# InternetMaximalism/intmax-zkp-core

Measured on NVIDIA B200. Metric: LDE+Merkle commit cells/s, higher is better.
Workload: dtype u64 (Goldilocks field, 32-bit IMAD/IADD3 limbs)

## Files before the change

intmax_zkp_core_b200/csrc/b200zkp.cu:

```cuda
#include "../../include/b200zkp.h"
#include "../../include/b200zkp_test.h"

#include <cuda_runtime.h>

#include <algorithm>
#include <cstdio>
#include <cstdlib>
#include <cstring>
#include <map>
#include <memory>
#include <mutex>
#include <optional>
#include <string>
#include <tuple>
#include <vector>

#include "merkle_kernels.cuh"
#include "ntt_kernels.cuh"
#include "eval_kernels.cuh"
#include "fri_kernels.cuh"
#include "perm_kernels.cuh"
#include "vanishing_kernels.cuh"
#include "host_plan.hpp"

using gl::u32;
using gl::u64;

static inline u64 gl_host_canon(u64 a) { return a >= hostgl::P ? a - hostgl::P : a; }

struct TwoLevel {
    u64* lo = nullptr;
    u64* hi = nullptr;
    u32 lo_bits = 0;
};

struct b200zkp_ctx {
    int device = 0;
    cudaStream_t stream = nullptr;
    bool own_stream = false;
    std::mutex mu;
    std::string err;
    u64 launches = 0;
    u64* wtab[2][ntt::MAX_PASS_BITS + 1] = {};
    std::map<u32, TwoLevel> tw[2];
    struct Images { const u64* img[ntt::MAX_PASSES] = {}; };
    std::map<std::tuple<u32, int, bool>, Images> twimg;
    std::map<std::pair<u32, u32>, const u64*> coset_scale;
    std::map<std::pair<u64, u32>, const u64*> power_scale;
    struct ZTables { const u64* strided = nullptr; const u64* final_ = nullptr; };
    std::map<std::pair<u32, u32>, ZTables> ztab_lde;
    std::map<u32, ZTables> ztab_inv;
    bool ntt_ct = true;
    bool ntt_tma = true;
    u32 ct_smem_set = 0;
    u32 sm_count = 0;
    u64 coop_leaf_rows = 2048;
    u64 coop_level_nodes = 2048;
    void* mailbox = nullptr;
    void* mailbox_dev = nullptr;
    u64* round_add = nullptr;
    std::multimap<size_t, void*> pool;
    size_t pool_bytes = 0;
    size_t live_bytes = 0;
    size_t pool_max_bytes = (size_t)16 << 30;
    std::vector<void*> table_allocs;
    cudaStream_t stream2 = nullptr;
    std::vector<cudaEvent_t> sync_events;
    bool timing = false;
    std::vector<cudaEvent_t> ev_free;
    struct Span { int stage; cudaEvent_t a, b; };
    std::vector<Span> spans;
};

struct StageTimer {
    b200zkp_ctx* c;
    int stage;
    cudaEvent_t a = nullptr;
    static cudaEvent_t get(b200zkp_ctx* c) {
        cudaEvent_t e = nullptr;
        if (!c->ev_free.empty()) { e = c->ev_free.back(); c->ev_free.pop_back(); }
        else if (cudaEventCreate(&e) != cudaSuccess) { (void)cudaGetLastError(); e = nullptr; }
        return e;
    }
    StageTimer(b200zkp_ctx* ctx, int st) : c(ctx), stage(st) {
        if (c->timing && (a = get(c))) cudaEventRecord(a, c->stream);
    }
    ~StageTimer() {
        if (!a) return;
        cudaEvent_t b = get(c);
        if (b) { cudaEventRecord(b, c->stream); c->spans.push_back({stage, a, b}); }
        else c->ev_free.push_back(a);
    }
};

struct Guard {
    b200zkp_ctx* c;
    explicit Guard(b200zkp_ctx* ctx) : c(ctx) { c->mu.lock(); cudaSetDevice(c->device); }
    ~Guard() { c->mu.unlock(); }
};

struct StreamScope {
    b200zkp_ctx* c;
    cudaStream_t saved;
    StreamScope(b200zkp_ctx* ctx, cudaStream_t s) : c(ctx), saved(ctx->stream) { c->stream = s; }
    ~StreamScope() { c->stream = saved; }
};

#define CUDA_TRY(ctx, expr)                                                                   \
    do {                                                                                      \
        cudaError_t e__ = (expr);                                                             \
        if (e__ != cudaSuccess) {                                                             \
            (ctx)->err = std::string(#expr) + ": " + cudaGetErrorString(e__);                 \
            (void)cudaGetLastError();                                                         \
            return e__ == cudaErrorMemoryAllocation ? B200ZKP_ERR_OOM : B200ZKP_ERR_CUDA;     \
        }                                                                                     \
    } while (0)
#define TRY(expr) do { int rc__ = (expr); if (rc__ != 0) return rc__; } while (0)
#define BAD(ctx, msg) do { (ctx)->err = (msg); return B200ZKP_ERR_BAD_ARG; } while (0)
#define LAUNCH_CHECK(ctx) do { (ctx)->launches++; CUDA_TRY(ctx, cudaGetLastError()); } while (0)

static void pool_drop(b200zkp_ctx* ctx) {
    for (auto& kv : ctx->pool) cudaFree(kv.second);
    ctx->pool.clear();
    ctx->pool_bytes = 0;
}

class DevBuf {
  public:
    DevBuf() = default;
    DevBuf(const DevBuf&) = delete;
    DevBuf& operator=(const DevBuf&) = delete;
    DevBuf(DevBuf&& o) noexcept : ctx_(o.ctx_), p_(o.p_), bytes_(o.bytes_) { o.p_ = nullptr; o.bytes_ = 0; }
    DevBuf& operator=(DevBuf&& o) noexcept {
        if (this != &o) { reset(); ctx_ = o.ctx_; p_ = o.p_; bytes_ = o.bytes_; o.p_ = nullptr; o.bytes_ = 0; }
        return *this;
    }
    ~DevBuf() { reset(); }

    u64* get() const { return (u64*)p_; }
    size_t bytes() const { return bytes_; }

    int alloc(b200zkp_ctx* ctx, size_t bytes) {
        reset();
        ctx_ = ctx;
        if (bytes == 0) return 0;
        void* p = nullptr;
        auto it = ctx->pool.find(bytes);
        if (it != ctx->pool.end()) {
            p = it->second; ctx->pool_bytes -= it->first; ctx->pool.erase(it);
        } else {
            cudaError_t e = cudaMalloc(&p, bytes);
            if (e == cudaErrorMemoryAllocation) {
                (void)cudaGetLastError();
                pool_drop(ctx);
                e = cudaMalloc(&p, bytes);
            }
            if (e != cudaSuccess) {
                ctx->err = std::string("cudaMalloc: ") + cudaGetErrorString(e);
                (void)cudaGetLastError();
                return e == cudaErrorMemoryAllocation ? B200ZKP_ERR_OOM : B200ZKP_ERR_CUDA;
            }
        }
        p_ = p; bytes_ = bytes;
        ctx->live_bytes += bytes;
        return 0;
    }
    int ensure(b200zkp_ctx* ctx, size_t bytes) { return bytes_ >= bytes ? 0 : alloc(ctx, bytes); }

    void reset() {
        if (!p_) return;
        ctx_->live_bytes -= bytes_;
        if (ctx_->pool.size() < 256 && ctx_->pool_bytes + bytes_ <= ctx_->pool_max_bytes) {
            ctx_->pool.emplace(bytes_, p_);
            ctx_->pool_bytes += bytes_;
        } else {
            cudaFree(p_);
        }
        p_ = nullptr; bytes_ = 0;
    }

  private:
    b200zkp_ctx* ctx_ = nullptr;
    void* p_ = nullptr;
    size_t bytes_ = 0;
};

struct b200zkp_batch {
    b200zkp_ctx* ctx;
    u32 n_log, k, rate_bits, cap_height, salt;
    DevBuf coeffs, lde, digests, cap;
};

struct b200zkp_tree {
    b200zkp_ctx* ctx;
    u64 n_leaves;
    u32 leaf_len, cap_height;
    DevBuf digests, cap;
};

static int d2h(b200zkp_ctx* ctx, void* dst, const void* src, size_t bytes) {
    if (!bytes) return 0;
    CUDA_TRY(ctx, cudaMemcpyAsync(dst, src, bytes, cudaMemcpyDeviceToHost, ctx->stream));
    CUDA_TRY(ctx, cudaStreamSynchronize(ctx->stream));
    return 0;
}
static int h2d(b200zkp_ctx* ctx, void* dst, const void* src, size_t bytes) {
    if (!bytes) return 0;
// ... 40 lines not shown
    auto it = cache.find(key);
    if (it == cache.end()) {
        typename Map::mapped_type t{};
        TRY(build(&t));
        it = cache.emplace(key, t).first;
    }
    *out = it->second;
    return 0;
}

static int get_tw(b200zkp_ctx* ctx, int dir, u32 n_log, TwoLevel* out) {
    return get_or_build(ctx->tw[dir], n_log, out, [&](TwoLevel* t) -> int {
        const u64 w = hostgl::root(n_log);
        std::vector<u64> lo, hi;
        t->lo_bits = hostgl::two_level_powers(dir ? hostgl::inv(w) : w, n_log, &lo, &hi);
        TRY(upload(ctx, lo, &t->lo));
        return upload(ctx, hi, &t->hi);
    });
}

static int fill_powers(b200zkp_ctx* ctx, u64 base, u32 bits, u64* dst) {
    std::vector<u64> lo, hi;
    const u32 lo_bits = hostgl::two_level_powers(base, bits, &lo, &hi);
    DevBuf d_lo, d_hi;
    TRY(d_lo.alloc(ctx, lo.size() * 8));
    TRY(d_hi.alloc(ctx, hi.size() * 8));
    TRY(h2d(ctx, d_lo.get(), lo.data(), d_lo.bytes()));
    TRY(h2d(ctx, d_hi.get(), hi.data(), d_hi.bytes()));
    const u64 n = (u64)1 << bits;
    ntt::build_powers_kernel<<<(unsigned)((n + 255) / 256), 256, 0, ctx->stream>>>(dst, n, d_lo.get(), d_hi.get(), lo_bits);
    LAUNCH_CHECK(ctx);
    CUDA_TRY(ctx, cudaStreamSynchronize(ctx->stream));
    return 0;
}

static int get_power_scale(b200zkp_ctx* ctx, u64 shift, u32 bits, const u64** out) {
    return get_or_build(ctx->power_scale, std::make_pair(shift, bits), out, [&](const u64** t) -> int {
        u64* d = nullptr;
        TRY(table_alloc(ctx, (u64)1 << bits, &d));
        *t = d;
        return fill_powers(ctx, shift, bits, d);
    });
}

static int get_coset_scale(b200zkp_ctx* ctx, u32 n_log, u32 rate_bits, const u64** out) {
    return get_or_build(ctx->coset_scale, std::make_pair(n_log, rate_bits), out, [&](const u64** t) -> int {
        const u64 n = (u64)1 << n_log;
        u64* d = nullptr;
        TRY(table_alloc(ctx, n << rate_bits, &d));
        for (u32 b = 0; b < (1u << rate_bits); b++)
            TRY(fill_powers(ctx, hostgl::coset_shift_of_block(n_log, rate_bits, b), n_log, d + (u64)b * n));
        *t = d;
        return 0;
    });
}

template <int B>
static void launch_pass_b(const ntt::PassParams& p, dim3 grid, cudaStream_t s) {
    switch (ntt::pass_mode(p)) {
        case ntt::MODE_MID_NATURAL: ntt::ntt_pass_kernel<B, ntt::MODE_MID_NATURAL><<<grid, ntt::threads_for(B), 0, s>>>(p); break;
        case ntt::MODE_MID_BITREV: ntt::ntt_pass_kernel<B, ntt::MODE_MID_BITREV><<<grid, ntt::threads_for(B), 0, s>>>(p); break;
        case ntt::MODE_FINAL_BITREV: ntt::ntt_pass_kernel<B, ntt::MODE_FINAL_BITREV><<<grid, ntt::threads_for(B), 0, s>>>(p); break;
        default: ntt::ntt_pass_kernel<B, ntt::MODE_FINAL_NATURAL><<<grid, ntt::threads_for(B), 0, s>>>(p); break;
    }
}
static int launch_pass(b200zkp_ctx* ctx, const ntt::PassParams& p, u32 B, u32 n_blk) {
    u64 T = (u64)ntt::tile_elems_for((int)B) >> B;
    u64 total_batches = (u64)p.ncols << (p.n_log - B);
    u64 blocks = (total_batches + T - 1) / T;
    if (blocks == 0 || n_blk == 0) return 0;
    if (blocks > 0x7fffffffull || n_blk > 65535) BAD(ctx, "transform too large for one launch");
    dim3 grid((unsigned)blocks, n_blk);
    switch (B) {
        case 1: launch_pass_b<1>(p, grid, ctx->stream); break;
        case 2: launch_pass_b<2>(p, grid, ctx->stream); break;
        case 3: launch_pass_b<3>(p, grid, ctx->stream); break;
        case 4: launch_pass_b<4>(p, grid, ctx->stream); break;
        case 5: launch_pass_b<5>(p, grid, ctx->stream); break;
        case 6: launch_pass_b<6>(p, grid, ctx->stream); break;
        case 7: launch_pass_b<7>(p, grid, ctx->stream); break;
        case 8: launch_pass_b<8>(p, grid, ctx->stream); break;
        case 9: launch_pass_b<9>(p, grid, ctx->stream); break;
        case 10: launch_pass_b<10>(p, grid, ctx->stream); break;
        default: BAD(ctx, "internal: bad pass width");
    }
    LAUNCH_CHECK(ctx);
    return 0;
}

static int launch_canon_copy(b200zkp_ctx* ctx, const u64* src, u64* dst, u64 count) {
    if (!count) return 0;
    ntt::canon_copy_kernel<<<(unsigned)((count + 255) / 256), 256, 0, ctx->stream>>>(src, dst, count);
    LAUNCH_CHECK(ctx);
    return 0;
}

static int get_twiddle_images(b200zkp_ctx* ctx, u32 n_log, int dir, bool bitrev_out, b200zkp_ctx::Images* out) {
    return get_or_build(ctx->twimg, std::make_tuple(n_log, dir, bitrev_out), out, [&](b200zkp_ctx::Images* im) -> int {
        ntt::TwiddleImageShape shapes[ntt::MAX_PASSES];
        u32 n_img = ntt::twiddle_images(n_log, shapes);
        if (!n_img) return 0;
        TwoLevel tw{};
        TRY(get_tw(ctx, dir, n_log, &tw));
        u64 n_inv = hostgl::inv(((u64)1 << n_log) % hostgl::P);
        for (u32 pi = 0; pi < n_img; pi++) {
            u64 count = (u64)1 << (shapes[pi].B + shapes[pi].C_log);
            u64* d = nullptr;
            TRY(table_alloc(ctx, count, &d));
            u64 f = (dir == 1 && pi == 0) ? n_inv : 0;
            ntt::build_twiddle_image_kernel<<<(unsigned)((count + 255) / 256), 256, 0, ctx->stream>>>(
                d, shapes[pi].B, shapes[pi].C_log, shapes[pi].shift, bitrev_out ? 1u : 0u, f, tw.lo, tw.hi, tw.lo_bits);
            LAUNCH_CHECK(ctx);
            im->img[pi] = d;
        }
        return 0;
    });
}

typedef CUresult (*TensorMapEncodeFn)(CUtensorMap*, CUtensorMapDataType, cuuint32_t, void*, const cuuint64_t*, const cuuint64_t*,
                                      const cuuint32_t*, const cuuint32_t*, CUtensorMapInterleave, CUtensorMapSwizzle,
                                      CUtensorMapL2promotion, CUtensorMapFloatOOBfill);
static TensorMapEncodeFn tensor_map_encoder() {
    static TensorMapEncodeFn fn = [] {
        void* p = nullptr;
        cudaDriverEntryPointQueryResult q;
        if (cudaGetDriverEntryPoint("cuTensorMapEncodeTiled", &p, cudaEnableDefault, &q) != cudaSuccess || q != cudaDriverEntryPointSuccess) {
            (void)cudaGetLastError();
            p = nullptr;
        }
        return (TensorMapEncodeFn)p;
    }();
    return fn;
}

static bool encode_tile_map(CUtensorMap* map, const u64* base, u32 B, u32 S, u32 C_log, u32 n_blk, u64 blk_stride, u32 ncols,
                            u64 col_stride) {
    TensorMapEncodeFn enc = tensor_map_encoder();
    if (!enc) return false;
    const u64 C = (u64)1 << C_log, rows = (u64)1 << B, A = (u64)1 << S;
    cuuint64_t dims[5] = {C, rows, A, n_blk ? n_blk : 1, ncols};
    cuuint64_t strides[4] = {C * 8, C * rows * 8, (blk_stride ? blk_stride : C * rows * A) * 8, col_stride * 8};
    cuuint32_t box[5] = {(cuuint32_t)(ntc::TILE >> B), (cuuint32_t)rows, 1, 1, 1};
    cuuint32_t estr[5] = {1, 1, 1, 1, 1};
    CUresult r = enc(map, CU_TENSOR_MAP_DATA_TYPE_UINT64, 5, (void*)base, dims, strides, box, estr, CU_TENSOR_MAP_INTERLEAVE_NONE,
                     CU_TENSOR_MAP_SWIZZLE_NONE, CU_TENSOR_MAP_L2_PROMOTION_L2_128B, CU_TENSOR_MAP_FLOAT_OOB_FILL_NONE);
    return r == CUDA_SUCCESS;
}

template <int B>
static int launch_ct_b(b200zkp_ctx* ctx, int kind, const ntc::PassParams& p, u64 grid, const CUtensorMap& tm_in, const CUtensorMap& tm_out,
                       const ntc::PullMaps* tm_src, const CUtensorMap* tm_copy, u32 pull_ctas_per_sm) {
    const void* fn = nullptr;
    u32 smem = 0;
    switch (kind) {
        case ntc::KIND_STRIDED: fn = (const void*)ntc::ct_pass_kernel<B, ntc::KIND_STRIDED>; smem = ntc::StridedSmem<B, false>::bytes; break;
        case ntc::KIND_STRIDED_LOOP: fn = (const void*)ntc::ct_pass_kernel<B, ntc::KIND_STRIDED_LOOP>; smem = ntc::StridedSmem<B, true>::bytes; break;
        case ntc::KIND_FINAL_INPLACE: fn = (const void*)ntc::ct_pass_kernel<B, ntc::KIND_FINAL_INPLACE>; smem = ntc::FinalSmem<B>::bytes; break;
        case ntc::KIND_PULL_LOOP: fn = (const void*)ntc::ct_pull_kernel<B>; smem = ntc::PullSmem<B>::bytes; break;
        default: fn = (const void*)ntc::ct_pass_kernel<B, ntc::KIND_FINAL_NATURAL>; smem = ntc::FinalSmem<B>::bytes; break;
    }
    const u32 bit = 1u << ((B - ntc::MIN_BITS) * 5 + kind);
    if (smem > 48 * 1024 && !(ctx->ct_smem_set & bit)) {
        CUDA_TRY(ctx, cudaFuncSetAttribute(fn, cudaFuncAttributeMaxDynamicSharedMemorySize, (int)smem));
        ctx->ct_smem_set |= bit;
    }
    void* args[5] = {(void*)&p, (void*)&tm_in, (void*)&tm_out, nullptr, nullptr};
    u32 total = (u32)grid;
    if (kind == ntc::KIND_PULL_LOOP) {
        args[1] = (void*)tm_src; args[2] = (void*)&tm_out; args[3] = (void*)tm_copy; args[4] = (void*)&total;
        if (!ctx->sm_count) {
            int sms = 0;
            CUDA_TRY(ctx, cudaDeviceGetAttribute(&sms, cudaDevAttrMultiProcessorCount, ctx->device));
            ctx->sm_count = (u32)std::max(1, sms);
        }
        grid = std::min<u64>(grid, (u64)std::max(1u, pull_ctas_per_sm) * ctx->sm_count);
    }
    CUDA_TRY(ctx, cudaLaunchKernel(fn, dim3((unsigned)grid), dim3(ntc::THREADS), args, smem, ctx->stream));
    ctx->launches++;
    return 0;
}

static int run_ct_plan(b200zkp_ctx* ctx, ntc::Plan& plan, cudaStream_t later_stream = nullptr, cudaEvent_t first_done = nullptr,
                       u32 pull_ctas_per_sm = 4) {
    cudaStream_t const first_stream = ctx->stream;
    std::optional<StreamScope> later;
    for (u32 pi = 0; pi < plan.n_passes; pi++) {
        if (pi == 1 && later_stream && later_stream != first_stream) {
            CUDA_TRY(ctx, cudaEventRecord(first_done, first_stream));
            CUDA_TRY(ctx, cudaStreamWaitEvent(later_stream, first_done, 0));
            later.emplace(ctx, later_stream);
        }
        ntc::PassParams& p = plan.pass[pi];
        const u32 B = plan.bits[pi];
        const int kind = plan.kind[pi];
        if (plan.grid[pi] > 0x7fffffffull) BAD(ctx, "transform too large for one launch");
        alignas(64) CUtensorMap tm_in, tm_out, tm_copy;
        alignas(64) ntc::PullMaps tm_src;
        memset(&tm_in, 0, sizeof tm_in); memset(&tm_out, 0, sizeof tm_out); memset(&tm_copy, 0, sizeof tm_copy);
        const bool pull = kind == ntc::KIND_PULL_LOOP;
        if (pull) memset(&tm_src, 0, sizeof tm_src);
        const u32 map_cols = p.col_run ? p.col_limit : p.ncols;
        if (p.use_tma) {
            const bool loop = kind == ntc::KIND_STRIDED_LOOP || pull;
            bool ok = ctx->ntt_tma && encode_tile_map(&tm_out, p.out, B, p.S, p.C_log, p.n_blk, p.out_blk_stride, map_cols, p.out_col_stride);
            if (ok && pull) {
                ok = encode_tile_map(&tm_copy, p.copy_out, B, p.S, p.C_log, 1, 0, map_cols, p.copy_col_stride);
                const u32 src_cols = ((p.col_limit + p.col_period - 1) / p.col_period) * p.col_run;
                for (u32 q = 0; ok && q < p.col_period / p.col_run; q++)
                    ok = encode_tile_map(&tm_src.m[q], p.src[q], B, p.S, p.C_log, 1, 0, src_cols, p.in_col_stride);
            } else if (ok) {
                ok = encode_tile_map(&tm_in, p.in, B, p.S, p.C_log, loop ? 1 : p.n_blk, loop ? 0 : p.in_blk_stride, map_cols, p.in_col_stride);
            }
            if (!ok) p.use_tma = 0;
        }
        switch (B) {
            case 5: TRY(launch_ct_b<5>(ctx, kind, p, plan.grid[pi], tm_in, tm_out, &tm_src, &tm_copy, pull_ctas_per_sm)); break;
            case 6: TRY(launch_ct_b<6>(ctx, kind, p, plan.grid[pi], tm_in, tm_out, &tm_src, &tm_copy, pull_ctas_per_sm)); break;
            case 7: TRY(launch_ct_b<7>(ctx, kind, p, plan.grid[pi], tm_in, tm_out, &tm_src, &tm_copy, pull_ctas_per_sm)); break;
            case 8: TRY(launch_ct_b<8>(ctx, kind, p, plan.grid[pi], tm_in, tm_out, &tm_src, &tm_copy, pull_ctas_per_sm)); break;
            default: BAD(ctx, "internal: bad pass width");
        }
    }
    return 0;
}

static int build_ztab(b200zkp_ctx* ctx, u32 n_log, int dir, const std::vector<u64>& shifts, u64 last_scale, bool natural,
                      b200zkp_ctx::ZTables* out) {
    TwoLevel tw{};
    TRY(get_tw(ctx, dir, n_log, &tw));
    std::vector<u64> spow((size_t)shifts.size() * n_log);
    for (size_t b = 0; b < shifts.size(); b++) {
        u64 x = shifts[b] % hostgl::P;
        for (u32 e = 0; e < n_log; e++) { spow[b * n_log + e] = x; x = hostgl::mul(x, x); }
    }
    DevBuf d_spow;
    TRY(d_spow.alloc(ctx, spow.size() * 8));
    TRY(h2d(ctx, d_spow.get(), spow.data(), d_spow.bytes()));
    const u64 count = ntc::ztab_entries(n_log), words = ntc::zfinal_words(n_log);
    u64 *d = nullptr, *f = nullptr;
    TRY(table_alloc(ctx, count * shifts.size(), &d));
    TRY(table_alloc(ctx, words * shifts.size(), &f));
    ntc::build_ztab_kernel<<<dim3((unsigned)((count + 255) / 256), (unsigned)shifts.size()), 256, 0, ctx->stream>>>(
        d, count, n_log, d_spow.get(), tw.lo, tw.hi, tw.lo_bits, last_scale);
    LAUNCH_CHECK(ctx);
    ntc::build_zfinal_kernel<<<dim3((unsigned)((words + 255) / 256), (unsigned)shifts.size()), 256, 0, ctx->stream>>>(
        f, words, n_log, ntc::last_pass_bits(n_log), natural ? 1u : 0u, d_spow.get(), tw.lo, tw.hi, tw.lo_bits, last_scale);
    LAUNCH_CHECK(ctx);
    CUDA_TRY(ctx, cudaStreamSynchronize(ctx->stream));
    out->strided = d;
    out->final_ = f;
    return 0;
}

static int get_ztab_lde(b200zkp_ctx* ctx, u32 n_log, u32 rate_bits, b200zkp_ctx::ZTables* out) {
    return get_or_build(ctx->ztab_lde, std::make_pair(n_log, rate_bits), out, [&](b200zkp_ctx::ZTables* t) {
        std::vector<u64> shifts;
        for (u32 b = 0; b < (1u << rate_bits); b++) shifts.push_back(hostgl::coset_shift_of_block(n_log, rate_bits, b));
        return build_ztab(ctx, n_log, 0, shifts, 0, false, t);
    });
}

static int get_ztab_inv(b200zkp_ctx* ctx, u32 n_log, b200zkp_ctx::ZTables* out) {
    return get_or_build(ctx->ztab_inv, n_log, out, [&](b200zkp_ctx::ZTables* t) {
        return build_ztab(ctx, n_log, 1, std::vector<u64>{1}, hostgl::inv(((u64)1 << n_log) % hostgl::P), true, t);
    });
}

static int run_transform(b200zkp_ctx* ctx, const u64* in, u64 in_stride, u64* out, u64 out_stride,
                         u64* scratch, u32 n_log, u32 ncols, int dir, bool bitrev_out,
                         const u64* scale, u64 scale_blk_stride, bool inverse_scale, bool canon_in,
                         u32 n_blk = 1, u64 out_blk_stride = 0) {
    if (ncols == 0) return 0;
    if (n_log == 0) {
        for (u32 blk = 0; blk < n_blk; blk++)
            for (u32 c = 0; c < ncols; c++)
                TRY(launch_canon_copy(ctx, in + c * in_stride, out + blk * out_blk_stride + c * out_stride, 1));
        return 0;
    }
    if (n_log > 32) BAD(ctx, "n_log exceeds the field's two-adicity (32)");
    if (!bitrev_out && n_log > (u32)ntt::MAX_PASS_BITS && !scratch) BAD(ctx, "scratch buffer required for multi-pass natural-order transforms");
    b200zkp_ctx::Images im;
    TRY(get_twiddle_images(ctx, n_log, dir, bitrev_out, &im));
    ntt::TransformTables tb{};
    tb.wtab = ctx->wtab[dir];
    for (u32 i = 0; i < ntt::MAX_PASSES; i++) tb.twimg[i] = im.img[i];
    tb.scale = scale;
    tb.scale_blk_stride = scale_blk_stride;
    u64 n_inv = hostgl::inv(((u64)1 << n_log) % hostgl::P);
    ntt::Plan plan;
    ntt::make_plan(&plan, in, in_stride, out, out_stride, scratch, n_log, ncols, tb, bitrev_out,
                   inverse_scale ? n_inv : 0, canon_in, 0, out_blk_stride);
    for (u32 pi = 0; pi < plan.n_passes; pi++) TRY(launch_pass(ctx, plan.pass[pi], plan.bits[pi], n_blk));
    return 0;
}

extern "C" const char* b200zkp_version(void) { return "b200zkp 0.1 (sm_100a)"; }

extern "C" int b200zkp_device_count(void) {
    int n = 0;
    cudaError_t e = cudaGetDeviceCount(&n);
    if (e != cudaSuccess) { (void)cudaGetLastError(); return B200ZKP_ERR_CUDA; }
    return n;
}

static int ctx_init_tables(b200zkp_ctx* ctx) {
    TRY(table_alloc(ctx, 360, &ctx->round_add));
    CUDA_TRY(ctx, cudaMemcpyFromSymbolAsync(ctx->round_add, poseidon_tables::ROUND_ADD, 360 * sizeof(u64), 0,
                                            cudaMemcpyDeviceToDevice, ctx->stream));
    for (int dir = 0; dir < 2; dir++)
        for (u32 B = 1; B <= (u32)ntt::MAX_PASS_BITS; B++) TRY(upload(ctx, hostgl::small_root_table(B, dir), &ctx->wtab[dir][B]));
    return 0;
}

extern "C" int b200zkp_ctx_create(int device, void* stream, b200zkp_ctx** out) {
// ... 1591 lines not shown
```

intmax_zkp_core_b200/csrc/ntt_ct_kernels.cuh:

```cuda
#pragma once
#include "goldilocks.cuh"

#ifndef B200ZKP_HOST_EMU
#include <cuda.h>
#endif

namespace ntc {

using gl::u32;
using gl::u64;

static constexpr int TILE = 2048;
static constexpr int THREADS = 256;
static constexpr int MIN_BITS = 5, MAX_BITS = 8;
static constexpr int MAX_LOOP_BLOCKS = 8;
static constexpr int MAX_SRC = 8;

enum Kind : int {
    KIND_STRIDED = 0,
    KIND_STRIDED_LOOP = 1,
    KIND_FINAL_INPLACE = 2,
    KIND_FINAL_NATURAL = 3,
    KIND_PULL_LOOP = 4,
};

struct PassParams {
    const u64* in;
    u64* out;
    u64 in_col_stride, out_col_stride;
    u64 in_blk_stride, out_blk_stride;
    u32 ncols, n_blk;
    u32 n_log;
    u32 S;
    u32 C_log;
    const u64* ztab;
    u64 ztab_blk_stride;
    u64 a_scale;
    u32 use_tma;
    u32 col_run, col_period, col0, col_limit, col_sel, col_src;
    const u64* src[MAX_SRC];
    u64* copy_out;
    u64 copy_col_stride;
};

GL_FN u32 map_column(const PassParams& p, u32 v, u32& q, u32& i) {
    if (p.col_run == 0) { q = 0; i = v; return v; }
    u32 phys;
    if (p.col_sel) phys = p.col0 + (v / p.col_run) * p.col_period + p.col_src * p.col_run + v % p.col_run;
    else phys = p.col0 + v;
    const u32 in_grp = phys % p.col_period;
    q = in_grp / p.col_run;
    i = (phys / p.col_period) * p.col_run + in_grp % p.col_run;
    return phys < p.col_limit ? phys : 0xFFFFFFFFu;
}

GL_FN u32 ulog2(u32 e) {
#ifdef B200ZKP_HOST_EMU
    u32 r = 0; while (e >>= 1) r++; return r;
#else
    return 31u - (u32)__clz((int)e);
#endif
}
GL_FN u32 bitrev_bits(u32 x, u32 bits) { return bits ? (gl::brev32(x) >> (32 - bits)) : 0; }

GL_FN u64 z_index(u64 prefix, u32 e) {
    const u32 u = ulog2(e);
    return (prefix << u) + (e ^ (1u << u));
}

GL_FN void butterfly(u64& a, u64& b, u64 z) {
    const u64 t = gl::canon_cc(gl::mul_nc(b, z));
    const u64 a0 = a;
    a = gl::add_nc(a0, t);
    b = gl::sub_nc(a0, t);
}

template <int A, bool SCALE>
GL_FN void ct_group(u64 (&x)[1 << A], const u64* __restrict__ tw, u32 u0, u32 gh, u64 a_scale) {
#pragma unroll
    for (int v = 0; v < A; v++) {
        const int half = (1 << A) >> (v + 1);
        u64 z[1 << (A - 1)];
#pragma unroll
        for (int q = 0; q < (1 << v); q++) z[q] = tw[(1u << (u0 + v)) + (gh << v) + q];
#pragma unroll
        for (int j = 0; j < (1 << A); j++) {
            if (j & half) continue;
            if (SCALE && v == A - 1) x[j] = gl::canon_cc(gl::mul_nc(x[j], a_scale));
            butterfly(x[j], x[j + half], z[j >> (A - v)]);
        }
    }
}

#ifdef B200ZKP_HOST_EMU
#define NTC_FOR_THREADS(tid) for (u32 tid = 0; tid < (u32)THREADS; tid++)
#define NTC_SYNC() do {} while (0)
#else
#define NTC_FOR_THREADS(tid) for (u32 tid = threadIdx.x, once__ = 1; once__; once__ = 0)
#define NTC_SYNC() __syncthreads()
#endif

template <int A, bool SCALE>
GL_FN void run_round(const u64* __restrict__ src, u64* __restrict__ dst, const u64* __restrict__ tw, u32 tw_pitch, u32 B,
                     u32 T_log, u32 pitch, u32 u0, u64 a_scale, u32 tid) {
    const u32 st_log = B - u0 - A;
    constexpr int UNITS = 8 >> A;
#pragma unroll
    for (int r = 0; r < UNITS; r++) {
        const u32 U = tid + r * THREADS;
        const u32 t = U & ((1u << T_log) - 1), w = U >> T_log;
        const u32 gl_ = w & ((1u << st_log) - 1), gh = w >> st_log;
        const u32 gbase = (gh << (st_log + A)) + gl_;
        u64 x[1 << A];
#pragma unroll
        for (int j = 0; j < (1 << A); j++) x[j] = src[(gbase + ((u32)j << st_log)) * pitch + t];
        ct_group<A, SCALE>(x, tw + t * tw_pitch, u0, gh, a_scale);
#pragma unroll
        for (int j = 0; j < (1 << A); j++) dst[(gbase + ((u32)j << st_log)) * pitch + t] = x[j];
    }
}

template <int B, bool SCALE>
GL_FN void run_rounds(const u64* first_src, u64* tile, const u64* tw, u32 tw_pitch, u32 T_log, u32 pitch, u64 a_scale) {
    u32 u0 = 0;
    const u64* src = first_src;
    if (B % 3 == 2) { NTC_FOR_THREADS(tid) { run_round<2, false>(src, tile, tw, tw_pitch, B, T_log, pitch, u0, a_scale, tid); } u0 += 2; src = tile; NTC_SYNC(); }
    if (B % 3 == 1) { NTC_FOR_THREADS(tid) { run_round<1, false>(src, tile, tw, tw_pitch, B, T_log, pitch, u0, a_scale, tid); } u0 += 1; src = tile; NTC_SYNC(); }
#pragma unroll 1
    for (int r = 0; r < B / 3 - 1; r++) {
        NTC_FOR_THREADS(tid) { run_round<3, false>(src, tile, tw, tw_pitch, B, T_log, pitch, u0, a_scale, tid); }
        u0 += 3; src = tile;
        NTC_SYNC();
    }
    NTC_FOR_THREADS(tid) { run_round<3, SCALE>(src, tile, tw, tw_pitch, B, T_log, pitch, u0, a_scale, tid); }
}

#ifndef B200ZKP_HOST_EMU
__device__ __forceinline__ u32 smem_u32(const void* p) { return (u32)__cvta_generic_to_shared(p); }
__device__ __forceinline__ void mbar_init(u64* bar, u32 count) {
    asm volatile("mbarrier.init.shared::cta.b64 [%0], %1;" ::"r"(smem_u32(bar)), "r"(count) : "memory");
}
__device__ __forceinline__ void fence_barrier_init() { asm volatile("fence.mbarrier_init.release.cluster;" ::: "memory"); }
__device__ __forceinline__ void fence_proxy_async() { asm volatile("fence.proxy.async.shared::cta;" ::: "memory"); }
__device__ __forceinline__ void mbar_expect_tx(u64* bar, u32 bytes) {
    asm volatile("mbarrier.arrive.expect_tx.shared::cta.b64 _, [%0], %1;" ::"r"(smem_u32(bar)), "r"(bytes) : "memory");
}
__device__ __forceinline__ void mbar_wait(u64* bar, u32 parity) {
    asm volatile(
        "{\n\t.reg .pred p;\n\t"
        "NTC_WAIT:\n\t"
        "mbarrier.try_wait.parity.shared::cta.b64 p, [%0], %1;\n\t"
        "@p bra NTC_DONE;\n\t"
        "bra NTC_WAIT;\n\t"
        "NTC_DONE:\n\t}" ::"r"(smem_u32(bar)), "r"(parity) : "memory");
}
__device__ __forceinline__ void tma_load_tile(void* dst, const CUtensorMap* map, u32 c0, u32 a, u32 blk, u32 col, u64* bar) {
    asm volatile("cp.async.bulk.tensor.5d.shared::cluster.global.mbarrier::complete_tx::bytes [%0], [%1, {%2, %3, %4, %5, %6}], [%7];"
                 ::"r"(smem_u32(dst)), "l"(map), "r"(c0), "r"(0u), "r"(a), "r"(blk), "r"(col), "r"(smem_u32(bar)) : "memory");
}
__device__ __forceinline__ void tma_store_tile(const CUtensorMap* map, u32 c0, u32 a, u32 blk, u32 col, const void* src) {
    asm volatile("cp.async.bulk.tensor.5d.global.shared::cta.bulk_group [%0, {%1, %2, %3, %4, %5}], [%6];"
                 ::"l"(map), "r"(c0), "r"(0u), "r"(a), "r"(blk), "r"(col), "r"(smem_u32(src)) : "memory");
}
__device__ __forceinline__ void bulk_load(void* dst, const void* src, u32 bytes, u64* bar) {
    asm volatile("cp.async.bulk.shared::cluster.global.mbarrier::complete_tx::bytes [%0], [%1], %2, [%3];"
                 ::"r"(smem_u32(dst)), "l"(src), "r"(bytes), "r"(smem_u32(bar)) : "memory");
}
__device__ __forceinline__ void tma_commit() { asm volatile("cp.async.bulk.commit_group;" ::: "memory"); }
template <int N>
__device__ __forceinline__ void tma_wait_read() { asm volatile("cp.async.bulk.wait_group.read %0;" ::"n"(N) : "memory"); }
template <int N>
__device__ __forceinline__ void tma_wait_all() { asm volatile("cp.async.bulk.wait_group %0;" ::"n"(N) : "memory"); }
#endif

template <int B, bool LOOP>
struct StridedSmem {
    static constexpr u32 NPTS = 1u << B;
    static constexpr u32 tiles = LOOP ? 3 : 1;
    static constexpr u32 sw_words = (LOOP ? (u32)MAX_LOOP_BLOCKS : 1u) * NPTS;
    static constexpr u32 bytes = tiles * TILE * 8 + sw_words * 8 + 16;
};

template <int B, bool LOOP, typename TMap, bool PULL = false>
GL_FN void strided_body(const PassParams& p, const TMap* tm_in, const TMap* tm_out, u64* smem, u32 bid, const TMap* tm_copy = nullptr) {
    static_assert(!PULL || LOOP, "a pull pass stages its tile apart from the work tiles");
    constexpr u32 NPTS = 1u << B;
    constexpr u32 T_log = 11 - B, T = 1u << T_log;
    constexpr u32 IT = TILE / THREADS;
    u64* const stage = smem;
    u64* const work0 = LOOP ? smem + TILE : smem;
    u64* const sw = smem + StridedSmem<B, LOOP>::tiles * TILE;
    u64* const bar = sw + StridedSmem<B, LOOP>::sw_words;

    const u32 V = LOOP ? p.ncols : p.ncols * p.n_blk;
    const u32 vcol = bid % V, tile_i = bid / V;
    u32 src_q, src_i;
    const u32 col = map_column(p, LOOP ? vcol : vcol / p.n_blk, src_q, src_i);
    if (col == 0xFFFFFFFFu) return;
    const u32 in_col = PULL ? src_i : col;
    const u32 blk_fixed = LOOP ? 0u : vcol % p.n_blk;
    const u32 tiles_per_a_log = p.C_log - T_log;
    const u32 a = tile_i >> tiles_per_a_log;
    const u32 c0 = (tile_i & ((1u << tiles_per_a_log) - 1)) << T_log;
    const u64 prefix = ((u64)1 << p.S) + a;
    const u64 elem0 = ((u64)a << (B + p.C_log)) + c0;
    const u64* __restrict__ in = (PULL ? p.src[src_q] : p.in) + (u64)in_col * p.in_col_stride + (u64)blk_fixed * p.in_blk_stride + elem0;
    (void)tm_in; (void)tm_out; (void)tm_copy; (void)bar;

#ifndef B200ZKP_HOST_EMU
    const bool tma = p.use_tma != 0;
    if (tma) {
        if (threadIdx.x == 0) { mbar_init(bar, 1); fence_barrier_init(); }
        __syncthreads();
        if (threadIdx.x == 0) {
            mbar_expect_tx(bar, TILE * 8);
            tma_load_tile(stage, PULL ? tm_in + src_q : tm_in, c0, a, blk_fixed, in_col, bar);
        }
    }
#else
    const bool tma = false;
#endif
    NTC_FOR_THREADS(tid) {
        const u32 nb = LOOP ? p.n_blk : 1u;
        for (u32 i = tid; i < nb * NPTS; i += THREADS) {
            const u32 b = LOOP ? i >> B : blk_fixed, e = i & (NPTS - 1);
            if (e) sw[i] = gl::ldg(p.ztab + (u64)b * p.ztab_blk_stride + z_index(prefix, e));
        }
        if (!tma) {
            u64 v[IT];
#pragma unroll
            for (u32 it = 0; it < IT; it++) {
                const u32 i = tid + it * THREADS;
                v[it] = in[((u64)(i >> T_log) << p.C_log) + (i & (T - 1))];
            }
#pragma unroll
            for (u32 it = 0; it < IT; it++) stage[tid + it * THREADS] = v[it];
            if (PULL) {
                u64* __restrict__ cp = p.copy_out + (u64)col * p.copy_col_stride + elem0;
#pragma unroll
                for (u32 it = 0; it < IT; it++) {
                    const u32 i = tid + it * THREADS;
                    cp[((u64)(i >> T_log) << p.C_log) + (i & (T - 1))] = v[it];
                }
            }
        }
    }
#ifndef B200ZKP_HOST_EMU
    if (tma) {
        mbar_wait(bar, 0);
        if (PULL && threadIdx.x == 0) { tma_store_tile(tm_copy, c0, a, 0, col, stage); tma_commit(); }
    }
#endif
    NTC_SYNC();

    const u32 n_loop = LOOP ? p.n_blk : 1u;
    for (u32 lb = 0; lb < n_loop; lb++) {
        const u32 blk = LOOP ? lb : blk_fixed;
        u64* const tile = LOOP ? work0 + (lb & 1) * TILE : work0;
#ifndef B200ZKP_HOST_EMU
        if (LOOP && tma && lb >= 2) { if (threadIdx.x == 0) tma_wait_read<1>(); __syncthreads(); }
#endif
        run_rounds<B, false>(LOOP ? stage : tile, tile, sw + (LOOP ? lb * NPTS : 0), 0, T_log, T, 0);
        u64* __restrict__ out = p.out + (u64)col * p.out_col_stride + (u64)blk * p.out_blk_stride + elem0;
#ifndef B200ZKP_HOST_EMU
        if (tma) {
            fence_proxy_async();
            __syncthreads();
            if (threadIdx.x == 0) { tma_store_tile(tm_out, c0, a, blk, col, tile); tma_commit(); }
            continue;
        }
#endif
        NTC_SYNC();
        NTC_FOR_THREADS(tid) {
#pragma unroll
            for (u32 it = 0; it < IT; it++) {
                const u32 i = tid + it * THREADS;
                out[((u64)(i >> T_log) << p.C_log) + (i & (T - 1))] = tile[i];
            }
        }
        NTC_SYNC();
    }
#ifndef B200ZKP_HOST_EMU
    if (tma && threadIdx.x == 0) tma_wait_read<0>();
#endif
}

template <int B>
struct FinalSmem {
    static constexpr u32 NPTS = 1u << B, T = (u32)TILE >> B;
    static constexpr u32 TP = T + 1, TWP = NPTS + 1;
    static constexpr u32 tw_words = T * TWP;
    static constexpr u32 bytes = (NPTS * TP + tw_words) * 8 + 16;
};

template <int B, bool NATURAL>
GL_FN void final_body(const PassParams& p, u64* smem, u32 bid) {
    constexpr u32 NPTS = 1u << B;
    constexpr u32 T_log = 11 - B, T = 1u << T_log, TP = FinalSmem<B>::TP, TWP = FinalSmem<B>::TWP;
    constexpr u32 IT = TILE / THREADS;
    u64* const tile = smem;
    u64* const swb = smem + NPTS * TP;
    u64* const bar = swb + FinalSmem<B>::tw_words;
    (void)bar;
    const u32 batches_log = p.n_log - B;
    const u32 V = p.ncols * p.n_blk;
    const u32 vcol = bid % V, tile_i = bid / V;
    u32 src_q, src_i;
    const u32 col = map_column(p, vcol / p.n_blk, src_q, src_i), blk = vcol % p.n_blk;
    if (col == 0xFFFFFFFFu) return;
    const u32 batch0 = tile_i << T_log;
    const u64* __restrict__ in = p.in + (u64)col * p.in_col_stride + (u64)blk * p.in_blk_stride;
    u64* __restrict__ out = p.out + (u64)col * p.out_col_stride + (u64)blk * p.out_blk_stride;
    const u64* __restrict__ ztile = p.ztab + (u64)blk * p.ztab_blk_stride + (u64)tile_i * FinalSmem<B>::tw_words;

#ifndef B200ZKP_HOST_EMU
    if (threadIdx.x == 0) { mbar_init(bar, 1); fence_barrier_init(); }
    __syncthreads();
    if (threadIdx.x == 0) {
        mbar_expect_tx(bar, FinalSmem<B>::tw_words * 8);
        bulk_load(swb, ztile, FinalSmem<B>::tw_words * 8, bar);
    }
#else
    for (u32 i = 0; i < FinalSmem<B>::tw_words; i++) swb[i] = ztile[i];
#endif
    NTC_FOR_THREADS(tid) {
        u64 v[IT];
#pragma unroll
        for (u32 it = 0; it < IT; it += 2) {
            const u32 i = 2 * (tid + (it / 2) * THREADS);
            const u32 b = i >> B, g = i & (NPTS - 1);
            const u32 a_b = NATURAL ? bitrev_bits(batch0 + b, batches_log) : batch0 + b;
#ifdef B200ZKP_HOST_EMU
            v[it] = in[((u64)a_b << B) + g]; v[it + 1] = in[((u64)a_b << B) + g + 1];
#else
            const ulonglong2 q = *reinterpret_cast<const ulonglong2*>(in + ((u64)a_b << B) + g);
            v[it] = q.x; v[it + 1] = q.y;
#endif
        }
#pragma unroll
        for (u32 it = 0; it < IT; it += 2) {
            const u32 i = 2 * (tid + (it / 2) * THREADS);
            const u32 b = i >> B, g = i & (NPTS - 1);
            tile[g * TP + b] = v[it];
            tile[(g + 1) * TP + b] = v[it + 1];
        }
    }
#ifndef B200ZKP_HOST_EMU
    mbar_wait(bar, 0);
#endif
    NTC_SYNC();

    if (p.a_scale) run_rounds<B, true>(tile, tile, swb, TWP, T_log, TP, p.a_scale);
    else run_rounds<B, false>(tile, tile, swb, TWP, T_log, TP, 0);
    NTC_SYNC();

    NTC_FOR_THREADS(tid) {
        if (NATURAL) {
#pragma unroll
            for (u32 it = 0; it < IT; it++) {
                const u32 i = tid + it * THREADS;
                const u32 tau = i & (T - 1), r = i >> T_log;
                const u32 g = bitrev_bits(r, B);
                out[((u64)r << batches_log) + batch0 + tau] = gl::canon_cc(tile[g * TP + tau]);
            }
        } else {
#pragma unroll
            for (u32 it = 0; it < IT; it += 2) {
                const u32 i = 2 * (tid + (it / 2) * THREADS);
                const u32 b = i >> B, g = i & (NPTS - 1);
                const u64 x0 = gl::canon_cc(tile[g * TP + b]), x1 = gl::canon_cc(tile[(g + 1) * TP + b]);
#ifdef B200ZKP_HOST_EMU
                out[((u64)(batch0 + b) << B) + g] = x0; out[((u64)(batch0 + b) << B) + g + 1] = x1;
#else
                *reinterpret_cast<ulonglong2*>(out + ((u64)(batch0 + b) << B) + g) = make_ulonglong2(x0, x1);
#endif
            }
        }
    }
}

#ifndef B200ZKP_HOST_EMU
template <int B, int KIND>
__global__ void __launch_bounds__(THREADS, 4)
ct_pass_kernel(const PassParams p, const __grid_constant__ CUtensorMap tm_in, const __grid_constant__ CUtensorMap tm_out) {
    extern __shared__ __align__(128) unsigned char ntc_smem_raw[];
    u64* smem = reinterpret_cast<u64*>(ntc_smem_raw);
    if (KIND == KIND_STRIDED) strided_body<B, false>(p, &tm_in, &tm_out, smem, blockIdx.x);
    else if (KIND == KIND_STRIDED_LOOP) strided_body<B, true>(p, &tm_in, &tm_out, smem, blockIdx.x);
    else if (KIND == KIND_FINAL_INPLACE) final_body<B, false>(p, smem, blockIdx.x);
    else final_body<B, true>(p, smem, blockIdx.x);
}

struct PullMaps { CUtensorMap m[MAX_SRC]; };
template <int B>
struct PullSmem {
    static constexpr u32 NPTS = 1u << B;
    static constexpr u32 sw_words = (u32)MAX_LOOP_BLOCKS * NPTS;
    static constexpr u32 bytes = 4 * TILE * 8 + sw_words * 8 + 32;
};

template <int B>
__device__ __forceinline__ void pull_decode(const PassParams& p, u32 bid, u32& col, u32& in_col, u32& q, u32& a, u32& c0) {
    constexpr u32 T_log = 11 - B;
    const u32 vcol = bid % p.ncols, tile_i = bid / p.ncols;
    u32 i;
    col = map_column(p, vcol, q, i);
    in_col = i;
    const u32 tiles_per_a_log = p.C_log - T_log;
    a = tile_i >> tiles_per_a_log;
    c0 = (tile_i & ((1u << tiles_per_a_log) - 1)) << T_log;
}

template <int B>
__global__ void __launch_bounds__(THREADS, 4)
ct_pull_kernel(const PassParams p, const __grid_constant__ PullMaps tm_src, const __grid_constant__ CUtensorMap tm_out,
               const __grid_constant__ CUtensorMap tm_copy, const u32 total) {
    extern __shared__ __align__(128) unsigned char ntc_smem_raw[];
    u64* const smem = reinterpret_cast<u64*>(ntc_smem_raw);
    if (!p.use_tma) {
        for (u32 bid = blockIdx.x; bid < total; bid += gridDim.x) {
            strided_body<B, true, CUtensorMap, true>(p, tm_src.m, &tm_out, smem, bid, &tm_copy);
            __syncthreads();
        }
        return;
    }
    constexpr u32 NPTS = 1u << B;
    constexpr u32 T_log = 11 - B, T = 1u << T_log;
    u64* const stage0 = smem;
    u64* const work0 = smem + 2 * TILE;
    u64* const sw = smem + 4 * TILE;
    u64* const bar = sw + PullSmem<B>::sw_words;
    if (blockIdx.x >= total) return;
    if (threadIdx.x == 0) { mbar_init(bar, 1); mbar_init(bar + 1, 1); fence_barrier_init(); }
    __syncthreads();
    u32 col, in_col, q, a, c0;
    if (threadIdx.x == 0) {
        pull_decode<B>(p, blockIdx.x, col, in_col, q, a, c0);
        mbar_expect_tx(bar, TILE * 8);
        tma_load_tile(stage0, &tm_src.m[q], c0, a, 0, in_col, bar);
    }
    u32 it = 0;
    for (u32 bid = blockIdx.x; bid < total; bid += gridDim.x, it++) {
        const u32 slot = it & 1;
        u64* const stage = stage0 + slot * TILE;
        if (threadIdx.x == 0 && bid + gridDim.x < total) {
            pull_decode<B>(p, bid + gridDim.x, col, in_col, q, a, c0);
            mbar_expect_tx(bar + (slot ^ 1), TILE * 8);
            tma_load_tile(stage0 + (slot ^ 1) * TILE, &tm_src.m[q], c0, a, 0, in_col, bar + (slot ^ 1));
        }
        pull_decode<B>(p, bid, col, in_col, q, a, c0);
        const u64 prefix = ((u64)1 << p.S) + a;
        for (u32 i = threadIdx.x; i < p.n_blk * NPTS; i += THREADS) {
            const u32 b = i >> B, e = i & (NPTS - 1);
            if (e) sw[i] = gl::ldg(p.ztab + (u64)b * p.ztab_blk_stride + z_index(prefix, e));
        }
        mbar_wait(bar + slot, (it >> 1) & 1);
        if (threadIdx.x == 0) { tma_store_tile(&tm_copy, c0, a, 0, col, stage); tma_commit(); }
        __syncthreads();
        for (u32 lb = 0; lb < p.n_blk; lb++) {
            u64* const tile = work0 + (lb & 1) * TILE;
            if (lb >= 2) { if (threadIdx.x == 0) tma_wait_read<1>(); __syncthreads(); }
            run_rounds<B, false>(stage, tile, sw + lb * NPTS, 0, T_log, T, 0);
            fence_proxy_async();
            __syncthreads();
            if (threadIdx.x == 0) { tma_store_tile(&tm_out, c0, a, lb, col, tile); tma_commit(); }
        }
        if (threadIdx.x == 0) tma_wait_read<0>();
        __syncthreads();
    }
}

__device__ __forceinline__ u64 z_entry(u64 i, u32 n_log, const u64* __restrict__ spow, const u64* __restrict__ lo,
                                       const u64* __restrict__ hi, u32 lo_bits, u64 last_scale) {
    if (!i) return 0;
    const u32 l = 63u - (u32)__clzll((long long)i);
    const u32 j = (u32)(i - ((u64)1 << l));
    const u64 e = (u64)bitrev_bits(j, l) << (n_log - 1 - l);
    const u64 w = gl::mul(gl::ldg(lo + (e & (((u64)1 << lo_bits) - 1))), gl::ldg(hi + (e >> lo_bits)));
    u64 r = gl::mul(w, gl::ldg(spow + (n_log - 1 - l)));
    if (last_scale && l == n_log - 1) r = gl::mul(r, last_scale);
    return r;
}
__global__ void build_ztab_kernel(u64* __restrict__ out, u64 count, u32 n_log, const u64* __restrict__ spow, const u64* __restrict__ lo,
                                  const u64* __restrict__ hi, u32 lo_bits, u64 last_scale) {
    const u64 i = (u64)blockIdx.x * blockDim.x + threadIdx.x;
    if (i >= count) return;
    out[(u64)blockIdx.y * count + i] = z_entry(i, n_log, spow + (u64)blockIdx.y * n_log, lo, hi, lo_bits, last_scale);
}
__global__ void build_zfinal_kernel(u64* __restrict__ out, u64 words, u32 n_log, u32 B, u32 natural, const u64* __restrict__ spow,
                                    const u64* __restrict__ lo, const u64* __restrict__ hi, u32 lo_bits, u64 last_scale) {
    const u64 x = (u64)blockIdx.x * blockDim.x + threadIdx.x;
    if (x >= words) return;
    const u32 T_log = 11 - B, TWP = (1u << B) + 1, S = n_log - B;
    const u64 tile_i = x / ((u64)TWP << T_log);
    const u32 rem = (u32)(x - tile_i * ((u64)TWP << T_log));
    const u32 b = rem / TWP, e = rem - b * TWP;
    u64 r = 0;
    if (e >= 1 && e < (1u << B)) {
        const u32 batch = (u32)(tile_i << T_log) + b;
        const u32 a_b = natural ? bitrev_bits(batch, S) : batch;
        r = z_entry(z_index(((u64)1 << S) + a_b, e), n_log, spow + (u64)blockIdx.y * n_log, lo, hi, lo_bits, last_scale);
    }
    out[(u64)blockIdx.y * words + x] = r;
}
#endif

}
```

Baseline: 1.097 billion.

## Specialize CT NTT kernels on column mapping, tune launch bounds, reroute butterfly add

Adds a compile-time MAPPED template parameter so column remapping logic is compiled out when no column set is used, reducing registers and integer work. Per-kind launch bounds are raised (6 blocks for strided, 5 for final) to push occupancy. The butterfly's modular add is replaced with inline PTX that routes part of the carry handling through a madc with a constant-memory zero, likely to shift work onto the multiply pipe. Higher min-blocks may force register spills, and the custom add must stay correct for Goldilocks reduction.

```diff
diff --git a/intmax_zkp_core_b200/csrc/b200zkp.cu b/intmax_zkp_core_b200/csrc/b200zkp.cu
--- a/intmax_zkp_core_b200/csrc/b200zkp.cu
+++ b/intmax_zkp_core_b200/csrc/b200zkp.cu
@@ -52,7 +52,7 @@
     std::map<u32, ZTables> ztab_inv;
     bool ntt_ct = true;
     bool ntt_tma = true;
-    u32 ct_smem_set = 0;
+    u64 ct_smem_set = 0;
     u32 sm_count = 0;
     u64 coop_leaf_rows = 2048;
     u64 coop_level_nodes = 2048;
@@ -399,14 +399,23 @@
                        const ntc::PullMaps* tm_src, const CUtensorMap* tm_copy, u32 pull_ctas_per_sm) {
     const void* fn = nullptr;
     u32 smem = 0;
+    const bool mapped = p.col_run != 0;
     switch (kind) {
-        case ntc::KIND_STRIDED: fn = (const void*)ntc::ct_pass_kernel<B, ntc::KIND_STRIDED>; smem = ntc::StridedSmem<B, false>::bytes; break;
-        case ntc::KIND_STRIDED_LOOP: fn = (const void*)ntc::ct_pass_kernel<B, ntc::KIND_STRIDED_LOOP>; smem = ntc::StridedSmem<B, true>::bytes; break;
-        case ntc::KIND_FINAL_INPLACE: fn = (const void*)ntc::ct_pass_kernel<B, ntc::KIND_FINAL_INPLACE>; smem = ntc::FinalSmem<B>::bytes; break;
+        case ntc::KIND_STRIDED:
+            fn = mapped ? (const void*)ntc::ct_pass_kernel<B, ntc::KIND_STRIDED, true> : (const void*)ntc::ct_pass_kernel<B, ntc::KIND_STRIDED, false>;
+            smem = ntc::StridedSmem<B, false>::bytes; break;
+        case ntc::KIND_STRIDED_LOOP:
+            fn = mapped ? (const void*)ntc::ct_pass_kernel<B, ntc::KIND_STRIDED_LOOP, true> : (const void*)ntc::ct_pass_kernel<B, ntc::KIND_STRIDED_LOOP, false>;
+            smem = ntc::StridedSmem<B, true>::bytes; break;
+        case ntc::KIND_FINAL_INPLACE:
+            fn = mapped ? (const void*)ntc::ct_pass_kernel<B, ntc::KIND_FINAL_INPLACE, true> : (const void*)ntc::ct_pass_kernel<B, ntc::KIND_FINAL_INPLACE, false>;
+            smem = ntc::FinalSmem<B>::bytes; break;
         case ntc::KIND_PULL_LOOP: fn = (const void*)ntc::ct_pull_kernel<B>; smem = ntc::PullSmem<B>::bytes; break;
-        default: fn = (const void*)ntc::ct_pass_kernel<B, ntc::KIND_FINAL_NATURAL>; smem = ntc::FinalSmem<B>::bytes; break;
-    }
-    const u32 bit = 1u << ((B - ntc::MIN_BITS) * 5 + kind);
+        default:
+            if (mapped) BAD(ctx, "internal: column set in natural order");
+            fn = (const void*)ntc::ct_pass_kernel<B, ntc::KIND_FINAL_NATURAL, false>; smem = ntc::FinalSmem<B>::bytes; break;
+    }
+    const u64 bit = 1ull << ((B - ntc::MIN_BITS) * 5 + kind + (mapped ? 20 : 0));
     if (smem > 48 * 1024 && !(ctx->ct_smem_set & bit)) {
         CUDA_TRY(ctx, cudaFuncSetAttribute(fn, cudaFuncAttributeMaxDynamicSharedMemorySize, (int)smem));
         ctx->ct_smem_set |= bit;
diff --git a/intmax_zkp_core_b200/csrc/ntt_ct_kernels.cuh b/intmax_zkp_core_b200/csrc/ntt_ct_kernels.cuh
--- a/intmax_zkp_core_b200/csrc/ntt_ct_kernels.cuh
+++ b/intmax_zkp_core_b200/csrc/ntt_ct_kernels.cuh
@@ -43,8 +43,14 @@
     u64 copy_col_stride;
 };
 
+template <bool MAPPED>
 GL_FN u32 map_column(const PassParams& p, u32 v, u32& q, u32& i) {
-    if (p.col_run == 0) { q = 0; i = v; return v; }
+#ifdef B200ZKP_HOST_EMU
+    const bool mapped = p.col_run != 0;
+#else
+    constexpr bool mapped = MAPPED;
+#endif
+    if (!mapped) { q = 0; i = v; return v; }
     u32 phys;
     if (p.col_sel) phys = p.col0 + (v / p.col_run) * p.col_period + p.col_src * p.col_run + v % p.col_run;
     else phys = p.col0 + v;
@@ -68,10 +74,31 @@
     return (prefix << u) + (e ^ (1u << u));
 }
 
+#ifdef B200ZKP_HOST_EMU
+GL_FN u64 add_nc_fma(u64 a, u64 c) { return gl::add_nc(a, c); }
+#else
+static __device__ __constant__ u32 FMA_ZERO = 0;
+GL_FN u64 add_nc_fma(u64 a, u64 c) {
+    u64 r;
+    asm("{\n\t"
+        ".reg .u32 l0, l1, m;\n\t"
+        ".reg .u64 t;\n\t"
+        "add.cc.u64 t, %1, %2;\n\t"
+        "madc.lo.u32 m, %3, %3, 0;\n\t"
+        "mov.b64 {l0, l1}, t;\n\t"
+        "sub.cc.u32 l0, l0, m;\n\t"
+        "subc.u32 l1, l1, 0;\n\t"
+        "add.u32 l1, l1, m;\n\t"
+        "mov.b64 %0, {l0, l1};\n\t"
+        "}" : "=l"(r) : "l"(a), "l"(c), "r"(FMA_ZERO));
+    return r;
+}
+#endif
+
 GL_FN void butterfly(u64& a, u64& b, u64 z) {
     const u64 t = gl::canon_cc(gl::mul_nc(b, z));
     const u64 a0 = a;
-    a = gl::add_nc(a0, t);
+    a = add_nc_fma(a0, t);
     b = gl::sub_nc(a0, t);
 }
 
@@ -181,7 +208,7 @@
     static constexpr u32 bytes = tiles * TILE * 8 + sw_words * 8 + 16;
 };
 
-template <int B, bool LOOP, typename TMap, bool PULL = false>
+template <int B, bool LOOP, typename TMap, bool PULL = false, bool MAPPED = PULL>
 GL_FN void strided_body(const PassParams& p, const TMap* tm_in, const TMap* tm_out, u64* smem, u32 bid, const TMap* tm_copy = nullptr) {
     static_assert(!PULL || LOOP, "a pull pass stages its tile apart from the work tiles");
     constexpr u32 NPTS = 1u << B;
@@ -195,7 +222,7 @@
     const u32 V = LOOP ? p.ncols : p.ncols * p.n_blk;
     const u32 vcol = bid % V, tile_i = bid / V;
     u32 src_q, src_i;
-    const u32 col = map_column(p, LOOP ? vcol : vcol / p.n_blk, src_q, src_i);
+    const u32 col = map_column<MAPPED>(p, LOOP ? vcol : vcol / p.n_blk, src_q, src_i);
     if (col == 0xFFFFFFFFu) return;
     const u32 in_col = PULL ? src_i : col;
     const u32 blk_fixed = LOOP ? 0u : vcol % p.n_blk;
@@ -293,7 +320,7 @@
     static constexpr u32 bytes = (NPTS * TP + tw_words) * 8 + 16;
 };
 
-template <int B, bool NATURAL>
+template <int B, bool NATURAL, bool MAPPED = false>
 GL_FN void final_body(const PassParams& p, u64* smem, u32 bid) {
     constexpr u32 NPTS = 1u << B;
     constexpr u32 T_log = 11 - B, T = 1u << T_log, TP = FinalSmem<B>::TP, TWP = FinalSmem<B>::TWP;
@@ -306,7 +333,7 @@
     const u32 V = p.ncols * p.n_blk;
     const u32 vcol = bid % V, tile_i = bid / V;
     u32 src_q, src_i;
-    const u32 col = map_column(p, vcol / p.n_blk, src_q, src_i), blk = vcol % p.n_blk;
+    const u32 col = map_column<MAPPED>(p, vcol / p.n_blk, src_q, src_i), blk = vcol % p.n_blk;
     if (col == 0xFFFFFFFFu) return;
     const u32 batch0 = tile_i << T_log;
     const u64* __restrict__ in = p.in + (u64)col * p.in_col_stride + (u64)blk * p.in_blk_stride;
@@ -380,15 +407,16 @@
 }
 
 #ifndef B200ZKP_HOST_EMU
-template <int B, int KIND>
-__global__ void __launch_bounds__(THREADS, 4)
+template <int B, int KIND, bool MAPPED>
+__global__ void __launch_bounds__(THREADS, KIND == KIND_STRIDED ? 6 : KIND == KIND_STRIDED_LOOP ? 4 : 5)
 ct_pass_kernel(const PassParams p, const __grid_constant__ CUtensorMap tm_in, const __grid_constant__ CUtensorMap tm_out) {
     extern __shared__ __align__(128) unsigned char ntc_smem_raw[];
     u64* smem = reinterpret_cast<u64*>(ntc_smem_raw);
-    if (KIND == KIND_STRIDED) strided_body<B, false>(p, &tm_in, &tm_out, smem, blockIdx.x);
-    else if (KIND == KIND_STRIDED_LOOP) strided_body<B, true>(p, &tm_in, &tm_out, smem, blockIdx.x);
-    else if (KIND == KIND_FINAL_INPLACE) final_body<B, false>(p, smem, blockIdx.x);
-    else final_body<B, true>(p, smem, blockIdx.x);
+    static_assert(!(MAPPED && KIND == KIND_FINAL_NATURAL), "column sets are stored in leaf order");
+    if (KIND == KIND_STRIDED) strided_body<B, false, CUtensorMap, false, MAPPED>(p, &tm_in, &tm_out, smem, blockIdx.x);
+    else if (KIND == KIND_STRIDED_LOOP) strided_body<B, true, CUtensorMap, false, MAPPED>(p, &tm_in, &tm_out, smem, blockIdx.x);
+    else if (KIND == KIND_FINAL_INPLACE) final_body<B, false, MAPPED>(p, smem, blockIdx.x);
+    else final_body<B, true, false>(p, smem, blockIdx.x);
 }
 
 struct PullMaps { CUtensorMap m[MAX_SRC]; };
@@ -404,7 +432,7 @@
     constexpr u32 T_log = 11 - B;
     const u32 vcol = bid % p.ncols, tile_i = bid / p.ncols;
     u32 i;
-    col = map_column(p, vcol, q, i);
+    col = map_column<true>(p, vcol, q, i);
     in_col = i;
     const u32 tiles_per_a_log = p.C_log - T_log;
     a = tile_i >> tiles_per_a_log;
```

After: 1.106 billion (median of 6 runs). About the same (+0.8%).
